# sulaimanvesal/PointCloudUDA

Measured on AMD Instinct MI355X. Metric: adversarial train-step images/sec (seg+3 discr) at 256x256, higher is better.
Workload: dtype bf16x3 MFMA (split-bf16, fp32 accumulate; fp32 storage); 1 GPU; MS-CMRSeg full UDA: UNet(PointNet head) + d1 + d2 + d4, 256x256x1, 4 classes; per_gpu_batch=32, global_batch=32, precision=bf16x3, parallelism=dp1, ranks_in_group=1, collective=none, streams=discriminators concurrent, d_target_forward=replayed from the adversarial pass of the same step, launch=eager (256 host cores for this rank)

## Files before the change

### pointcloududa_amd/csrc/conv_host.h

```cpp
#pragma once
#include <stdlib.h>
#include <string.h>
#include "conv_igemm.h"

static const int LDS_HARD = 160 * 1024;

static inline bool geom_ok(const pcuda_conv_geom* g) {
  if (!g || g->n <= 0 || g->cin <= 0 || g->cout <= 0 || g->k <= 0 || g->stride <= 0 || g->dil <= 0 || g->pad < 0)
    return false;
  if (g->k * g->k > IG_MAX_TAPS) return false;
  const int oh = (g->in_h + 2 * g->pad - g->dil * (g->k - 1) - 1) / g->stride + 1;
  const int ow = (g->in_w + 2 * g->pad - g->dil * (g->k - 1) - 1) / g->stride + 1;
  if (oh != g->out_h || ow != g->out_w || oh <= 0 || ow <= 0) return false;
  if (g->in_up && ((g->in_h & 1) || (g->in_w & 1))) return false;
  return true;
}

static inline bool src_ok(const pcuda_src* s, int c) {
  if (!s || !s->p1 || s->c1 <= 0 || s->c1 > c) return false;
  if (s->c1 < c && !s->p2) return false;
  return true;
}
static inline bool dst_ok(const pcuda_dst* d, int c) {
  if (!d || !d->p1 || d->c1 <= 0 || d->c1 > c) return false;
// ... 75 lines not shown

static inline int tile_width_candidates(int lw, int tile_px, int* out) {
  int n = 0;
  for (int t = 8; t <= 256 && t <= tile_px; t <<= 1) out[n++] = t;
  for (int parts = 1; parts <= 4; ++parts) {
    const int t = (lw + parts - 1) / parts;
    if (t >= 4 && t <= 256 && t <= tile_px) {
      bool dup = false;
      for (int i = 0; i < n; ++i) dup |= out[i] == t;
      if (!dup) out[n++] = t;
    }
  }
  return n;
}


static inline bool fast_src_ok(const pcuda_src* x, int cin) {
  const long long lim = 1ll << 30;
  const int c1 = x->c1 < cin ? x->c1 : cin;
  if (c1 < cin && (c1 & 31)) return false;
  if ((long long)(c1 + 32) * x->sc1 * 4 >= lim) return false;
  if (c1 < cin && (long long)(cin - c1 + 32) * x->sc2 * 4 >= lim) return false;
  return true;
}

static inline bool fast_dst_ok(const pcuda_dst* y, int cout) {
  const long long lim = 1ll << 30;
  const int c1 = y->c1 < cout ? y->c1 : cout;
  if (c1 < cout && (c1 & 7)) return false;
  if ((long long)(c1 + 64) * y->sc1 * 4 >= lim) return false;
  if (c1 < cout && (long long)(cout - c1 + 64) * y->sc2 * 4 >= lim) return false;
  return true;
}

struct IgemmPlan {
  int npb, tw, th, tiles_x, tiles_y, ih_t, iw_t, clamp, x_cap, tg;
  size_t lds;
  int fat;
  int w8;
  int te;
};

static inline bool te_dst_ok(const pcuda_dst* y, int cout, int out_w, int lw, int tw, int ox_mul, int ox_off) {
  if (ox_mul != 1 || ox_off != 0 || (tw & 3) || (out_w & 3) || (lw & 3)) return false;
  if (((uintptr_t)y->p1 & 15) || (y->sc1 & 3) || (y->sn1 & 3)) return false;
  if (y->c1 < cout && (((uintptr_t)y->p2 & 15) || (y->sc2 & 3) || (y->sn2 & 3))) return false;
  return true;
}


struct IgemmParams;
struct PackParams;
bool ap_layer_ok(const pcuda_conv_geom* g, int rows, int red, int prec);
size_t ap_layer_packed_bytes(int rows, int red);
bool ap_fill_pack(PackParams& p, const float* w, unsigned char* out, int rows, int red, long long s_row, long long s_red,
                  const TapSet& taps);
int ap_launch_pack(const float* w, unsigned char* out, int rows, int red, long long s_row, long long s_red, const TapSet& taps,
                   hipStream_t s);
bool ap_map_ok(int n, int h, int w, int rows);
int ap_tiles(int n, int h, int w);
int ap_try_launch(const IgemmParams& p, const TapSet& taps, const unsigned char* image, hipStream_t s, int* rc);

bool rs_layer_ok(const pcuda_conv_geom* g, int rows, int red, int prec);
bool rs_map_ok(int n, int h, int w);
int rs_tiles(int n, int h, int w);
int rs_try_launch(const IgemmParams& p, int prec, const TapSet& taps, hipStream_t s, int* rc);

int direct_fwd_tiles(const pcuda_conv_geom* g);
int direct_forward(const pcuda_conv_geom* g, int prec, const pcuda_src* x, const void* packed_w, long long w_lo_off,
                   const float* bias, float slope, const pcuda_dst* y, float* bn_partials, hipStream_t s, int* rc);
int direct_dgrad_tiles(const pcuda_conv_geom* g);
int direct_dgrad(const pcuda_conv_geom* g, int prec, const pcuda_src* dy, const void* packed_w_dgrad, const pcuda_dst* dx,
                 int accumulate, hipStream_t s, int* rc, const float* red_a = nullptr, long long red_sn = 0,
                 long long red_sc = 0, const float* red_mean = nullptr, const float* red_invstd = nullptr,
                 float* red = nullptr);
size_t direct_wgrad_workspace(const pcuda_conv_geom* g);
int direct_wgrad(const pcuda_conv_geom* g, const pcuda_src* x, const float* dz, long long dz_sn, long long dz_sc, float* dw,
                 float* db, int accumulate, void* workspace, hipStream_t s, int* rc);
int direct_d1_dgrad(const pcuda_conv_geom* g, int prec, const pcuda_src* dy, const void* packed_w_dgrad, const pcuda_dst* dx,
                    int accumulate, size_t cls_elems, hipStream_t s, int* rc);
size_t direct_d1_wgrad_workspace(const pcuda_conv_geom* g);
int direct_d1_wgrad(const pcuda_conv_geom* g, const pcuda_src* x, const float* dz, long long dz_sn, long long dz_sc, float* dw,
                    float* db, int accumulate, void* workspace, hipStream_t s, int* rc);
int launch_wgrad_reduce_taps(const float* partial, long long numel, int ksplit, float* dw, int accumulate, int ntaps,
                             const float* db_partial, long long nb, float* db, hipStream_t s);
size_t wgrad3r_workspace(const pcuda_conv_geom* g);
int wgrad3r_try(const pcuda_conv_geom* g, int prec, const pcuda_src* x, const float* dy, long long dy_sn, long long dy_sc,
                float* dw, float* db, int accumulate, void* workspace, hipStream_t s, pcuda_reduce_job* defer, int* rc);
size_t wgrad1_workspace(const pcuda_conv_geom* g);
int wgrad1_try(const pcuda_conv_geom* g, int prec, const pcuda_src* x, const float* dy, long long dy_sn, long long dy_sc,
               float* dw, float* db, int accumulate, void* workspace, hipStream_t s, pcuda_reduce_job* defer, int* rc);
size_t wgrad3_workspace(const pcuda_conv_geom* g);
int wgrad3_try(const pcuda_conv_geom* g, int prec, const pcuda_src* x, const float* dy, long long dy_sn, long long dy_sc,
               float* dw, float* db, int accumulate, void* workspace, hipStream_t s, pcuda_reduce_job* defer, int* rc);
int launch_wgrad_reduce(const float* partial, long long numel, int ksplit, float* dw, int accumulate, const float* db_partial,
                        long long nb, float* db, hipStream_t s);
int direct_d1_forward(const pcuda_conv_geom* g, int prec, const pcuda_src* x, const void* packed_w, const float* bias,
                      float slope, const pcuda_dst* y, float* bn_partials, hipStream_t s, int* rc);
int direct_d5_forward(const pcuda_conv_geom* g, int prec, const pcuda_src* x, const void* packed_w, const float* bias,
                      float slope, const pcuda_dst* y, float* bn_partials, hipStream_t s, int* rc);
```

### pointcloududa_amd/csrc/conv_wgrad.hip

```cpp
#include "conv_igemm.h"
#include "conv_host.h"

__global__ __launch_bounds__(1024) void wgrad_reduce_kernel(const float* __restrict__ partial, long long numel,
                                                           int ksplit, float* __restrict__ dw, int accumulate,
                                                           int ntaps, const float* __restrict__ db_partial,
                                                           long long nb, float* __restrict__ db) {
  __shared__ float sh[16][64];
  const int lane = threadIdx.x & 63, kg = threadIdx.x >> 6, nkg = blockDim.x >> 6;
  const long long nblk_w = (numel + 63) / 64;
  long long blk = blockIdx.x;
  if (blk >= nblk_w) {
    blk -= nblk_w; partial = db_partial; numel = nb; dw = db; ntaps = 1;
  }
  const long long i = blk * 64 + lane;
  float s = 0.f;
  if (i < numel) {
    int k = kg;
    for (; k + 7 * nkg < ksplit; k += 8 * nkg) {
      float v[8];
#pragma unroll
      for (int u = 0; u < 8; ++u) v[u] = partial[(long long)(k + u * nkg) * numel + i];
#pragma unroll
      for (int u = 0; u < 8; ++u) s += v[u];
    }
    for (; k < ksplit; k += nkg) s += partial[(long long)k * numel + i];
  }
  sh[kg][lane] = s;
  __syncthreads();
  if (kg == 0 && i < numel) {
    float t = 0.f;
    for (int q = 0; q < nkg; ++q) t += sh[q][lane];
    long long o = i;
    if (ntaps > 1) {
      const long long cc = numel / ntaps;
      const long long tt = i / cc, r = i - tt * cc;
      o = r * ntaps + tt;
    }
    dw[o] = accumulate ? dw[o] + t : t;
  }
}

int launch_wgrad_reduce_taps(const float* partial, long long numel, int ksplit, float* dw, int accumulate, int ntaps,
                             const float* db_partial, long long nb, float* db, hipStream_t s) {
  int nkg = 1;
  while (nkg < 16 && nkg * 2 <= ksplit) nkg <<= 1;
  const unsigned nblk = (unsigned)cdiv(numel, 64) + (db ? (unsigned)cdiv(nb, 64) : 0u);
  hipLaunchKernelGGL(wgrad_reduce_kernel, dim3(nblk), dim3(64 * nkg), 0, s, partial, numel, ksplit, dw, accumulate, ntaps,
                     db_partial, db ? nb : 0, db);
  PCUDA_CHECK_LAUNCH("wgrad_reduce_kernel");
  return PCUDA_OK;
}
int launch_wgrad_reduce(const float* partial, long long numel, int ksplit, float* dw, int accumulate, const float* db_partial,
                        long long nb, float* db, hipStream_t s) {
  return launch_wgrad_reduce_taps(partial, numel, ksplit, dw, accumulate, 1, db_partial, nb, db, s);
}

struct ReduceJobs {
  int n;
  int first_block[PCUDA_REDUCE_MAX_JOBS + 1];
  pcuda_reduce_job j[PCUDA_REDUCE_MAX_JOBS];
};

__global__ __launch_bounds__(1024) void wgrad_reduce_batch_kernel(const ReduceJobs jobs) {
  __shared__ float sh[16][64];
  int lo = 0, hi = jobs.n - 1;
  while (lo < hi) {
    const int mid = (lo + hi + 1) >> 1;
    if (jobs.first_block[mid] <= (int)blockIdx.x) lo = mid; else hi = mid - 1;
  }
  const pcuda_reduce_job& jb = jobs.j[lo];
  const float* partial = jb.partial;
  long long numel = jb.numel;
  float* dw = jb.dw;
  int ntaps = jb.ntaps;
  const int ksplit = jb.ksplit, nkg = jb.nkg;
  const int lane = threadIdx.x & 63, kg = threadIdx.x >> 6;
  const long long nblk_w = (numel + 63) / 64;
  long long blk = (int)blockIdx.x - jobs.first_block[lo];
  if (blk >= nblk_w) { blk -= nblk_w; partial = jb.db_partial; numel = jb.nb; dw = jb.db; ntaps = 1; }
  const long long i = blk * 64 + lane;
  float s = 0.f;
  if (i < numel && kg < nkg) {
    int k = kg;
    for (; k + 7 * nkg < ksplit; k += 8 * nkg) {
      float v[8];
#pragma unroll
      for (int u = 0; u < 8; ++u) v[u] = partial[(long long)(k + u * nkg) * numel + i];
#pragma unroll
      for (int u = 0; u < 8; ++u) s += v[u];
    }
    for (; k < ksplit; k += nkg) s += partial[(long long)k * numel + i];
  }
  sh[kg][lane] = s;
  __syncthreads();
  if (kg == 0 && i < numel) {
    float t = 0.f;
    for (int q = 0; q < nkg; ++q) t += sh[q][lane];
    long long o = i;
    if (ntaps > 1) {
      const long long cc = numel / ntaps;
      const long long tt = i / cc, r = i - tt * cc;
      o = r * ntaps + tt;
    }
    dw[o] = jb.accumulate ? dw[o] + t : t;
  }
}

extern "C" int pcuda_wgrad_reduce_batch(const pcuda_reduce_job* host_jobs, int njobs, pcuda_stream_t s) {
  if (!host_jobs || njobs < 0) PCUDA_FAIL(PCUDA_E_BADARG, "wgrad_reduce_batch: bad arguments");
  int done = 0;
  while (done < njobs) {
    ReduceJobs jobs;
    jobs.n = 0;
    int blocks = 0;
    for (; done < njobs && jobs.n < PCUDA_REDUCE_MAX_JOBS; ++done) {
      const pcuda_reduce_job& jb = host_jobs[done];
      if (jb.ksplit <= 0) continue;
      if (!jb.partial || !jb.dw || jb.numel <= 0 || jb.nkg < 1 || jb.nkg > 16 || (jb.db && !jb.db_partial))
        PCUDA_FAIL(PCUDA_E_BADARG, "wgrad_reduce_batch: bad job %d", done);
      jobs.first_block[jobs.n] = blocks;
      jobs.j[jobs.n++] = jb;
      blocks += (int)cdiv(jb.numel, 64) + (jb.db ? (int)cdiv(jb.nb, 64) : 0);
    }
    if (jobs.n == 0) break;
    jobs.first_block[jobs.n] = blocks;
    ProfScope prof(PCUDA_FAM_POINTWISE, 0.0, (hipStream_t)s, "wgrad reduce batch");
    hipLaunchKernelGGL(wgrad_reduce_batch_kernel, dim3(blocks), dim3(1024), 0, (hipStream_t)s, jobs);
    PCUDA_CHECK_LAUNCH("wgrad_reduce_batch_kernel");
  }
  return PCUDA_OK;
}

namespace {

struct WgradPlan {
  int co_blks, co_tile, n_co_tiles, n_chunks, tap_groups, taps_per_group, tw, th, tiles_x, tiles_y, ksplit;
  int ih_t, iw_t;
};

WgradPlan plan_wgrad(const pcuda_conv_geom* g) {
  WgradPlan w;
  w.co_blks = ig_co_blks(g->cout);
  w.co_tile = 32 * w.co_blks;
  w.n_co_tiles = cdiv(g->cout, w.co_tile);
  w.n_chunks = cdiv(g->cin, 32);
  const int ntaps = g->k * g->k;
  w.tap_groups = ntaps <= 16 ? 1 : cdiv(ntaps, 9);
  w.taps_per_group = cdiv(ntaps, w.tap_groups);
  {
    int cand[16];
    const int nc = tile_width_candidates(g->out_w, 128, cand);
    long long best_key = -1;
    w.tw = 32; w.th = 4;
    for (int ci = 0; ci < nc; ++ci) {
      const int tw = cand[ci], th = 128 / tw;
      if (th < 1) continue;
      const int span = (g->k - 1) * g->dil;
      const long long halo = (long long)((th - 1) * g->stride + span + 1) * ((tw - 1) * g->stride + span + 1);
      {
        const long long ih = (th - 1) * g->stride + span + 1, iw = (tw - 1) * g->stride + span + 1;
        const long long clipped = (ih < g->in_h ? ih : g->in_h) * (iw < g->in_w ? iw : g->in_w) + 1;
        const long long cap = halo < clipped ? halo : clipped;
        if (cap * IG_REC_BYTES * 2 + (long long)w.co_tile * WG_ZROW * 2 > (long long)LDS_HARD) continue;
      }
      const long long ih2 = (th - 1) * g->stride + span + 1, iw2 = (tw - 1) * g->stride + span + 1;
      const long long clipped2 = (ih2 < g->in_h ? ih2 : g->in_h) * (iw2 < g->in_w ? iw2 : g->in_w) + 1;
      const long long staged = (clipped2 * 2 <= halo) ? clipped2 : halo;
      const long long key = ((long long)cdiv(g->out_w, tw) * cdiv(g->out_h, th) << 24) + (staged > 768 ? (1ll << 22) : 0) +
                            ((tw & 31) ? (1ll << 20) : 0) + halo;
      if (best_key < 0 || key < best_key) { best_key = key; w.tw = tw; w.th = th; }
    }
  }
  const int TW = w.tw, TH = w.th;
  w.tiles_x = cdiv(g->out_w, TW);
  w.tiles_y = cdiv(g->out_h, TH);
  const int span = (g->k - 1) * g->dil;
  w.ih_t = (TH - 1) * g->stride + span + 1;
  w.iw_t = (TW - 1) * g->stride + span + 1;
  const long long ntiles = (long long)g->n * w.tiles_x * w.tiles_y;
  const int base = w.n_co_tiles * w.n_chunks * w.tap_groups;
  static int tgt32 = -1;
  if (tgt32 < 0) { const char* e = getenv("PCUDA_WG_BLOCKS32"); tgt32 = e ? atoi(e) : 768; }
  static int tgt64 = -1;
  if (tgt64 < 0) { const char* e = getenv("PCUDA_WG_BLOCKS64"); tgt64 = e ? atoi(e) : 1024; }
  static int tgt1 = -1;
  if (tgt1 < 0) { const char* e = getenv("PCUDA_WG_BLOCKS1"); tgt1 = e ? atoi(e) : 256; }
  bool one_per_cu = false;
  {
    const long long full = (long long)w.ih_t * w.iw_t;
    const long long clipped = (long long)(w.ih_t < g->in_h ? w.ih_t : g->in_h) * (w.iw_t < g->in_w ? w.iw_t : g->in_w) + 1;
    const size_t zb = (size_t)w.co_tile * WG_ZROW * 2;
    bool clamp = clipped * 2 <= full;
    if (!clamp && (size_t)full * IG_REC_BYTES * 2 + zb > (size_t)LDS_HARD) clamp = true;
    one_per_cu = (size_t)(clamp ? clipped : full) * IG_REC_BYTES * 2 + zb > (size_t)LDS_HARD / 2;
  }
  long long ks = (one_per_cu ? tgt1 : (w.co_blks == 1 ? tgt32 : tgt64)) / base;
  if (ks < 1) ks = 1;
  if (ks > ntiles) ks = ntiles;
  const long long welems = (long long)g->cout * g->cin * ntaps;
  while (ks > 1 && ks * welems * 4 > (64ll << 20)) ks >>= 1;
  if (ks >= 8) ks &= ~7ll;
  w.ksplit = (int)ks;
  return w;
}

}

extern "C" size_t pcuda_conv2d_wgrad_workspace_size(const pcuda_conv_geom* g) {
  if (!geom_ok(g)) return 0;
  WgradPlan w = plan_wgrad(g);
// ... 45 lines not shown
               pcuda_conv2d_wgrad_workspace_size(g));
  {
    int rc;
    if (direct_wgrad(g, x, dy, dy_sn, dy_sc, dw, db, accumulate, workspace, s, &rc)) return rc;
    if (direct_d1_wgrad(g, x, dy, dy_sn, dy_sc, dw, db, accumulate, workspace, s, &rc)) return rc;
    if (wgrad3r_try(g, prec, x, dy, dy_sn, dy_sc, dw, db, accumulate, workspace, s, defer, &rc)) return rc;
    if (wgrad3_try(g, prec, x, dy, dy_sn, dy_sc, dw, db, accumulate, workspace, s, defer, &rc)) return rc;
    if (wgrad1_try(g, prec, x, dy, dy_sn, dy_sc, dw, db, accumulate, workspace, s, defer, &rc)) return rc;
  }
  const bool x3 = prec == PCUDA_PREC_BF16X3;
  WgradPlan w = plan_wgrad(g);
  TapSet t = fwd_taps(g);
  WgradParams p;
  memset(&p, 0, sizeof(p));
  p.x = *x; p.cin = g->cin;
  p.in_h = g->in_h; p.in_w = g->in_w; p.in_shift = g->in_up ? 1 : 0; p.in_row = g->in_w >> p.in_shift;
  p.dz = dy; p.dz_sn = dy_sn; p.dz_sc = dy_sc;
  p.cout = g->cout; p.out_h = g->out_h; p.out_w = g->out_w;
  p.stride = g->stride;
  p.ntaps = w.taps_per_group; p.ntaps_total = t.n; p.tap_groups = w.tap_groups;
  memcpy(p.dy, t.dy, sizeof(p.dy));
  memcpy(p.dx, t.dx, sizeof(p.dx));
  p.dy_min = t.dy_min; p.dx_min = t.dx_min;
  p.ih_t = w.ih_t; p.iw_t = w.iw_t;
  p.tw = w.tw; p.th = w.th; p.tmagic = 65536 / w.tw + 1; p.tiles_x = w.tiles_x; p.tiles_y = w.tiles_y; p.n = g->n;
  p.ksplit = w.ksplit; p.n_co_tiles = w.n_co_tiles; p.n_chunks = w.n_chunks;
  p.partial = (float*)workspace;
  {
    static int dbg = -1;
    if (dbg < 0) { const char* e = getenv("PCUDA_DBG"); dbg = e ? atoi(e) : 0; }
    p.dbg = dbg;
  }
  p.tw16 = ((w.tw & 15) == 0 && w.tw * w.th == 128) ? 1 : 0;
  p.aligned4 = ((g->out_w & 7) == 0 && (w.tw & 7) == 0 && (dy_sn & 3) == 0 && (dy_sc & 3) == 0 && (((uintptr_t)dy) & 15) == 0 &&
                ((long long)g->cout * dy_sc + (long long)g->out_h * g->out_w) * 4 < (1ll << 30)) ? 1 : 0;
  const long long welems = (long long)g->cout * g->cin * t.n;
  float* dbp = db ? (float*)workspace + (size_t)w.ksplit * welems : nullptr;

  const int full = w.ih_t * w.iw_t;
  const int clipped = (w.ih_t < g->in_h ? w.ih_t : g->in_h) * (w.iw_t < g->in_w ? w.iw_t : g->in_w) + 1;
  const size_t mul = x3 ? 2 : 1;
  const size_t zb = (size_t)w.co_tile * WG_ZROW * mul;
  bool clamp = clipped * 2 <= full;
  if (!clamp && (size_t)full * IG_REC_BYTES * mul + zb > (size_t)LDS_HARD) clamp = true;
  const int x_cap = clamp ? clipped : full;
  const size_t lds = (size_t)x_cap * IG_REC_BYTES * mul + zb;
  if (lds > (size_t)LDS_HARD) PCUDA_FAIL(PCUDA_E_UNSUPPORTED, "conv2d_wgrad: tile %dx%d does not fit LDS", w.ih_t, w.iw_t);
  const dim3 grid(w.n_co_tiles * w.n_chunks * w.tap_groups, w.ksplit);
  {
    static int noxcd = -1;
    if (noxcd < 0) { const char* e = getenv("PCUDA_WG_NOXCD"); noxcd = (e && atoi(e)) ? 1 : 0; }
    const long long nblk = (long long)grid.x * grid.y;
    p.xcd_items = (!noxcd && nblk >= 16 && (nblk & 7) == 0) ? (int)(nblk / 8) : 0;
    static int nointer = -1;
    if (nointer < 0) { const char* e = getenv("PCUDA_WG_NOINTER"); nointer = (e && atoi(e)) ? 1 : 0; }
    p.xcd_slices = (p.xcd_items && !nointer && (w.ksplit & 7) == 0) ? w.ksplit / 8 : 0;
  }
  {
    const double flops = 2.0 * g->n * (double)g->out_h * g->out_w * g->cout * (double)g->cin * t.n;
    char tag[160];
    static int nopipe = -1;
    if (nopipe < 0) { const char* e = getenv("PCUDA_NOPIPE"); nopipe = (e && atoi(e)) ? 1 : 0; }
    int pf = (nopipe || !fast_src_ok(x, g->cin)) ? 0 : (x_cap <= 256 ? 1 : (x_cap <= 768 ? 3 : 0));
    static int now8 = -1;
    if (now8 < 0) { const char* e = getenv("PCUDA_WG_NO8"); now8 = (e && atoi(e)) ? 1 : 0; }
    if (!now8 && pf > 0 && w.taps_per_group > 9 && x_cap <= 1024) pf = 100 + (x_cap <= 512 ? 1 : 2);
    {
      static int noxq = -1;
      if (noxq < 0) { const char* e = getenv("PCUDA_NOXQ"); noxq = e ? atoi(e) : 0; }
      const int slots = pf >= 100 ? pf - 100 : pf, per = pf >= 100 ? 128 : 64;
      const int ih = clamp ? (w.ih_t < g->in_h ? w.ih_t : g->in_h) : w.ih_t;
      const int in_w_phys = g->in_up ? g->in_w / 2 : g->in_w;
      p.xq = (!noxq && slots > 0 && !g->in_up && (in_w_phys & 3) == 0 && (ih * ((w.iw_t + 6) / 4) + per - 1) / per <= slots) ? 1 : 0;
    }
    snprintf(tag, sizeof(tag), "wgrad n%d cin%d cout%d %dx%d k%d s%d d%d ksplit%d clamp%d pf%d lds%zu", g->n, g->cin,
             g->cout, g->out_h, g->out_w, g->k, g->stride, g->dil, w.ksplit, clamp ? 1 : 0, pf, lds);
    ProfScope prof(PCUDA_FAM_CONV_WGRAD, flops, s, tag);
    int rc;
    const int taps_max = w.taps_per_group <= 1 ? 1 : w.taps_per_group <= 9 ? 9 : 16;
    rc = x3 ? wgrad_dispatch_x3(p, w.co_blks, clamp, taps_max, pf, x_cap, lds, dbp, grid, s)
            : wgrad_dispatch_bf16(p, w.co_blks, clamp, taps_max, pf, x_cap, lds, dbp, grid, s);
    if (rc) return rc;
  }
  {
    int nkg = 1;
    while (nkg < 16 && nkg * 2 <= w.ksplit) nkg <<= 1;
    if (defer) {
      defer->partial = (const float*)workspace; defer->numel = welems; defer->ksplit = w.ksplit; defer->nkg = nkg;
      defer->dw = dw; defer->accumulate = accumulate; defer->ntaps = t.n;
      defer->db_partial = (const float*)dbp; defer->nb = db ? g->cout : 0; defer->db = db;
      return PCUDA_OK;
    }
    const unsigned nblk = (unsigned)cdiv(welems, 64) + (db ? (unsigned)cdiv(g->cout, 64) : 0u);
    hipLaunchKernelGGL(wgrad_reduce_kernel, dim3(nblk), dim3(64 * nkg), 0, s, (const float*)workspace, welems, w.ksplit,
                       dw, accumulate, t.n, (const float*)dbp, (long long)(db ? g->cout : 0), db);
    PCUDA_CHECK_LAUNCH("wgrad_reduce_kernel");
  }
  return PCUDA_OK;
}
```

### pointcloududa_amd/csrc/conv_wgrad1.hip

```cpp
#include "conv_device.h"
#include "conv_host.h"

namespace {

struct W1Params {
  pcuda_src x;
  int cin, cout, n;
  int hw;
  const float* dz; long long dz_sn, dz_sc;
  float* partial;
  float* db_partial;
  int steps_per_wg;
  int wgs_per_image;
  int n_ci_tiles, tiles;
  int xcd;
};

template <int NB>
struct W1Raw {
  f32x4 v[NB][2];
};

template <bool X3, int CO_B, int CI_B>
__global__ __launch_bounds__(256, 2) void wgrad1_kernel(const W1Params p) {
// ... 168 lines not shown
  static int off = -1;
  if (off < 0) { const char* e = getenv("PCUDA_NO_WGRAD1"); off = (e && atoi(e)) ? 1 : 0; }
  if (off) return false;
  const long long hw = (long long)g->in_h * g->in_w;
  return g->k == 1 && g->stride == 1 && g->pad == 0 && !g->in_up && (hw & 15) == 0 && hw < (1ll << 28) && g->cin >= 16;
}

W1Plan w1_plan(const pcuda_conv_geom* g) {
  W1Plan w;
  w.co_b = g->cout > 32 ? 2 : 1;
  w.ci_b = g->cin > 64 ? 3 : (g->cin > 32 ? 2 : 1);
  w.n_co_tiles = cdiv(g->cout, 32 * w.co_b);
  w.n_ci_tiles = cdiv(g->cin, 32 * w.ci_b);
  const int tiles = w.n_co_tiles * w.n_ci_tiles;
  const long long spi = (long long)g->in_h * g->in_w / 16, total = spi * g->n;
  static int tgt = -1;
  if (tgt < 0) { const char* e = getenv("PCUDA_WG1_BLOCKS"); tgt = e ? atoi(e) : 768; }
  long long want = tgt / tiles;
  const long long welems = (long long)g->cout * g->cin;
  const long long in_bytes = total * 16 * (g->cin + g->cout) * 4;
  long long cap = in_bytes / 8;
  if (cap < (8ll << 20)) cap = 8ll << 20;
  if (want * welems * 4 > cap) want = cap / (welems * 4);
  if (want > total / 8) want = total / 8;
  if (want < 1) want = 1;
  long long d = cdiv(total, want);
  if (d > spi) d = spi;
  while (spi % d) ++d;
  w.steps_per_wg = (int)d;
  w.wgs_per_image = (int)(spi / d);
  w.slices = w.wgs_per_image * g->n;
  return w;
}

}

size_t wgrad1_workspace(const pcuda_conv_geom* g) {
  if (!w1_geom(g)) return 0;
  const W1Plan w = w1_plan(g);
  return ((size_t)w.slices * g->cout * g->cin + (size_t)w.slices * g->cout) * sizeof(float) + 256;
}

int wgrad1_try(const pcuda_conv_geom* g, int prec, const pcuda_src* x, const float* dy, long long dy_sn, long long dy_sc,
               float* dw, float* db, int accumulate, void* workspace, hipStream_t s, pcuda_reduce_job* defer, int* rc) {
  if (!w1_geom(g)) return 0;
  auto al = [](const void* q, long long sn, long long sc) { return q == nullptr || ((((uintptr_t)q) & 15) == 0 && (sn & 3) == 0 && (sc & 3) == 0); };
  const int c1 = x->c1 < g->cin ? x->c1 : g->cin;
  if (!al(x->p1, x->sn1, x->sc1) || (c1 < g->cin && !al(x->p2, x->sn2, x->sc2)) || !al(dy, dy_sn, dy_sc)) return 0;
  const bool x3 = prec == PCUDA_PREC_BF16X3;
  const W1Plan w = w1_plan(g);
  W1Params p;
  memset(&p, 0, sizeof(p));
  p.x = *x; p.x.c1 = c1;
  p.cin = g->cin; p.cout = g->cout; p.n = g->n; p.hw = g->in_h * g->in_w;
  p.dz = dy; p.dz_sn = dy_sn; p.dz_sc = dy_sc;
  const long long welems = (long long)g->cout * g->cin;
  p.partial = (float*)workspace;
  p.db_partial = db ? (float*)workspace + (size_t)w.slices * welems : nullptr;
  p.steps_per_wg = w.steps_per_wg; p.wgs_per_image = w.wgs_per_image;
  p.n_ci_tiles = w.n_ci_tiles; p.tiles = w.n_co_tiles * w.n_ci_tiles;
  const long long nwg = (long long)p.tiles * w.slices;
  if (nwg >= (1ll << 31)) return 0;
  p.xcd = (nwg >= 16 && (nwg & 7) == 0) ? 1 : 0;
  {
    char tag[160];
    snprintf(tag, sizeof(tag), "wgrad1 n%d cin%d cout%d %dx%d k1 slices%d steps%d tile%dx%d", g->n, g->cin, g->cout, g->in_h,
             g->in_w, w.slices, w.steps_per_wg, 32 * w.co_b, 32 * w.ci_b);
    ProfScope prof(PCUDA_FAM_CONV_WGRAD, 2.0 * g->n * (double)p.hw * g->cout * (double)g->cin, s, tag);
    const dim3 grid((unsigned)nwg);
#define W1_LAUNCH(X3_, CO_, CI_) hipLaunchKernelGGL((wgrad1_kernel<X3_, CO_, CI_>), grid, dim3(256), 0, s, p)
#define W1_CI(X3_, CO_)                                                \
  do {                                                                 \
    if (w.ci_b == 3) W1_LAUNCH(X3_, CO_, 3);                           \
    else if (w.ci_b == 2) W1_LAUNCH(X3_, CO_, 2);                      \
    else W1_LAUNCH(X3_, CO_, 1);                                       \
  } while (0)
    if (x3) { if (w.co_b == 2) W1_CI(true, 2); else W1_CI(true, 1); }
    else { if (w.co_b == 2) W1_CI(false, 2); else W1_CI(false, 1); }
#undef W1_CI
#undef W1_LAUNCH
    hipError_t e = hipGetLastError();
    if (e != hipSuccess) { pcuda_set_error("wgrad1_kernel: %s", hipGetErrorString(e)); *rc = PCUDA_E_LAUNCH; return 1; }
  }
  int nkg = 1;
  while (nkg < 16 && nkg * 2 <= w.slices) nkg <<= 1;
  if (defer) {
    defer->partial = (const float*)workspace; defer->numel = welems; defer->ksplit = w.slices; defer->nkg = nkg;
    defer->dw = dw; defer->accumulate = accumulate; defer->ntaps = 1;
    defer->db_partial = (const float*)p.db_partial; defer->nb = db ? g->cout : 0; defer->db = db;
    *rc = PCUDA_OK;
    return 1;
  }
  *rc = launch_wgrad_reduce_taps((const float*)workspace, welems, w.slices, dw, accumulate, 1, (const float*)p.db_partial,
                                 db ? g->cout : 0, db, s);
  return 1;
}
```

### pointcloududa_amd/csrc/conv_wgrad3.hip

```cpp
#include "conv_device.h"
#include "conv_host.h"

namespace {

constexpr int W3_TW = 32, W3_TH = 4;
constexpr int W3_XW = 40;
constexpr int W3_XROWS = W3_TH + 2;
constexpr int W3_XREC = W3_XW * W3_XROWS;
constexpr int W3_XPLANE = W3_XREC * IG_REC_BYTES;
constexpr int W3_ITEMS = W3_XROWS * (W3_XW / 4);

struct W3Params {
  pcuda_src x;
  int cin, H, W;
  const float* dz; long long dz_sn, dz_sc;
  int cout;
  int tiles_x, tiles_y, n;
  int ksplit, n_chunks;
  float* partial;
  float* db_partial;
  int base, xcd;
  int dbg;
};

// ... 293 lines not shown
  return true;
}

W3Plan w3_plan(const pcuda_conv_geom* g) {
  W3Plan w;
  w.rb = 2;
  w.kh = 1;
  w.n_co_tiles = g->cout / (32 * w.rb);
  w.n_chunks = g->cin / 32;
  w.tiles_x = g->out_w / W3_TW;
  w.tiles_y = g->out_h / W3_TH;
  const long long ntiles = (long long)g->n * w.tiles_x * w.tiles_y;
  const int base = w.n_co_tiles * w.n_chunks;
  static int tgt = -1;
  if (tgt < 0) { const char* e = getenv("PCUDA_WG3_BLOCKS"); tgt = e ? atoi(e) : 1024; }
  long long ks = tgt / base;
  if (ks < 1) ks = 1;
  if (ks > ntiles) ks = ntiles;
  const long long welems = (long long)g->cout * g->cin * 9;
  while (ks > 1 && ks * w.kh * welems * 4 > (64ll << 20)) ks >>= 1;
  if (ks >= 8) ks &= ~7ll;
  w.ksplit = (int)ks;
  return w;
}

}

size_t wgrad3_workspace(const pcuda_conv_geom* g) {
  if (g->k != 3 || g->stride != 1 || g->dil != 1 || g->pad != 1 || g->in_up || (g->out_w % W3_TW) || (g->out_h % W3_TH) ||
      (g->cout & 63) || (g->cin & 31))
    return 0;
  const W3Plan w = w3_plan(g);
  return ((size_t)w.ksplit * w.kh * g->cout * g->cin * 9 + (size_t)w.ksplit * w.kh * g->cout) * sizeof(float) + 256;
}

int wgrad3_try(const pcuda_conv_geom* g, int prec, const pcuda_src* x, const float* dy, long long dy_sn, long long dy_sc,
               float* dw, float* db, int accumulate, void* workspace, hipStream_t s, pcuda_reduce_job* defer, int* rc) {
  if (!w3_eligible(g, x, dy, dy_sn, dy_sc)) return 0;
  const bool x3 = prec == PCUDA_PREC_BF16X3;
  const W3Plan w = w3_plan(g);
  W3Params p;
  memset(&p, 0, sizeof(p));
  p.x = *x; p.cin = g->cin; p.H = g->in_h; p.W = g->in_w;
  p.dz = dy; p.dz_sn = dy_sn; p.dz_sc = dy_sc; p.cout = g->cout;
  p.tiles_x = w.tiles_x; p.tiles_y = w.tiles_y; p.n = g->n;
  p.ksplit = w.ksplit; p.n_chunks = w.n_chunks;
  {
    static int dbg = -1;
    if (dbg < 0) { const char* e = getenv("PCUDA_W3DBG"); dbg = e ? atoi(e) : 0; }
    p.dbg = dbg;
  }
  const int slices = w.ksplit * w.kh;
  const long long welems = (long long)g->cout * g->cin * 9;
  p.partial = (float*)workspace;
  p.db_partial = db ? (float*)workspace + (size_t)slices * welems : nullptr;
  const size_t lds = (size_t)(x3 ? 2 : 1) * (W3_XPLANE + 32 * w.rb * WG_ZROW);
  p.base = w.n_co_tiles * w.n_chunks;
  {
    static int noxcd = -1;
    if (noxcd < 0) { const char* e = getenv("PCUDA_W3_NOXCD"); noxcd = (e && atoi(e)) ? 1 : 0; }
    p.xcd = (!noxcd && (w.ksplit % 8) == 0) ? 1 : 0;
  }
  const dim3 grid(p.base * w.ksplit);
  {
    char tag[160];
    snprintf(tag, sizeof(tag), "wgrad3 n%d cin%d cout%d %dx%d k3 s1 d1 ksplit%d rb%d lds%zu", g->n, g->cin, g->cout, g->out_h,
             g->out_w, w.ksplit, w.rb, lds);
    ProfScope prof(PCUDA_FAM_CONV_WGRAD, 2.0 * g->n * (double)g->out_h * g->out_w * g->cout * (double)g->cin * 9, s, tag);
#define W3_LAUNCH(X3_, RB_, KH_)                                                                                       \
  do {                                                                                                                  \
    auto kern = wgrad3_kernel<X3_, RB_, KH_>;                                                                          \
    if (lds > 48 * 1024) {                  \
      hipError_t e = hipFuncSetAttribute((const void*)kern, hipFuncAttributeMaxDynamicSharedMemorySize, (int)LDS_HARD); \
      if (e != hipSuccess) { pcuda_set_error("wgrad3: cannot raise dynamic LDS: %s", hipGetErrorString(e)); *rc = PCUDA_E_LAUNCH; return 1; } \
    }                                                                                                                   \
    hipLaunchKernelGGL(kern, grid, dim3(64 * RB_ * 2 * KH_), lds, s, p);                                                \
  } while (0)
    if (x3) W3_LAUNCH(true, 2, 1);
    else W3_LAUNCH(false, 2, 1);
#undef W3_LAUNCH
    hipError_t e = hipGetLastError();
    if (e != hipSuccess) { pcuda_set_error("wgrad3_kernel: %s", hipGetErrorString(e)); *rc = PCUDA_E_LAUNCH; return 1; }
  }
  int nkg = 1;
  while (nkg < 16 && nkg * 2 <= slices) nkg <<= 1;
  if (defer) {
    defer->partial = (const float*)workspace; defer->numel = welems; defer->ksplit = slices; defer->nkg = nkg;
    defer->dw = dw; defer->accumulate = accumulate; defer->ntaps = 9;
    defer->db_partial = (const float*)p.db_partial; defer->nb = db ? g->cout : 0; defer->db = db;
    *rc = PCUDA_OK;
    return 1;
  }
  *rc = launch_wgrad_reduce_taps((const float*)workspace, welems, slices, dw, accumulate, 9, (const float*)p.db_partial,
                                 db ? g->cout : 0, db, s);
  return 1;
}
```

### pointcloududa_amd/csrc/conv_wgrad3r.hip

```cpp
#include <type_traits>

#include "conv_device.h"
#include "conv_host.h"

namespace {

struct W3RParams {
  pcuda_src x;
  int cin, cout, n, H, W;
  const float* dz; long long dz_sn, dz_sc;
  float* partial;
  float* db_partial;
  int n_ci_tiles, tiles;
  int strips;
  int rsplit;
  int npairs;
  int pairs_per_slice;
  int xcd;
  int dbg;
};

struct RowF {
  uint4 f[3][2];
};
// ... 267 lines not shown
  if (maxc < 0) { const char* e = getenv("PCUDA_W3R_MAXC"); maxc = e ? atoi(e) : 128; }
  static int upmaxc = -1;
  if (upmaxc < 0) { const char* e = getenv("PCUDA_W3R_UPMAXC"); upmaxc = e ? atoi(e) : 512; }
  const int mc = (g->in_up && upmaxc > maxc) ? upmaxc : maxc;
  const bool shape = g->k == 3 && g->stride == 1 && g->pad == 1 && g->dil == 1 && (g->in_w & 31) == 0 && g->in_h >= 4 &&
                     (!g->in_up || (g->in_h & 1) == 0) &&
                     g->cin >= 16 && g->cin <= mc && g->cout <= mc && (long long)g->in_h * g->in_w < (1ll << 28);
  if (!shape || mode >= 2) return shape;
  if (g->in_up) return g->cin <= upmaxc && g->cout <= upmaxc;
  if (g->in_h >= 128 && g->in_w >= 128) return true;
  return g->cin != g->cout && g->cin <= 64 && g->cout <= 64 && g->in_h >= 64;
}

W3RPlan w3r_plan(const pcuda_conv_geom* g) {
  W3RPlan w;
  w.n_co_tiles = cdiv(g->cout, 32);
  w.n_ci_tiles = cdiv(g->cin, 32);
  const int tiles = w.n_co_tiles * w.n_ci_tiles;
  w.strips = g->in_w / 32;
  w.rsplit = 1;
  while ((long long)g->n * w.strips * w.rsplit * tiles < 256 && g->in_h / (w.rsplit * 2) >= 32) w.rsplit *= 2;
  w.npairs = g->n * w.strips * w.rsplit;
  static int tgt = -1;
  if (tgt < 0) { const char* e = getenv("PCUDA_W3R_BLOCKS"); tgt = e ? atoi(e) : 512; }
  long long want = tgt / tiles;
  const long long welems = (long long)g->cout * g->cin * 9;
  if (want * welems * 4 > (32ll << 20)) want = (32ll << 20) / (welems * 4);
  if (want < 1) want = 1;
  if (want > w.npairs) want = w.npairs;
  w.pairs_per_slice = cdiv(w.npairs, (int)want);
  w.slices = cdiv(w.npairs, w.pairs_per_slice);
  return w;
}

}

size_t wgrad3r_workspace(const pcuda_conv_geom* g) {
  if (!w3r_geom(g)) return 0;
  const W3RPlan w = w3r_plan(g);
  return ((size_t)w.slices * g->cout * g->cin * 9 + (size_t)w.slices * g->cout) * sizeof(float) + 256;
}

int wgrad3r_try(const pcuda_conv_geom* g, int prec, const pcuda_src* x, const float* dy, long long dy_sn, long long dy_sc,
                float* dw, float* db, int accumulate, void* workspace, hipStream_t s, pcuda_reduce_job* defer, int* rc) {
  if (!w3r_geom(g)) return 0;
  auto al = [](const void* q, long long sn, long long sc) { return q == nullptr || ((((uintptr_t)q) & 15) == 0 && (sn & 3) == 0 && (sc & 3) == 0); };
  const int c1 = x->c1 < g->cin ? x->c1 : g->cin;
  if (!al(x->p1, x->sn1, x->sc1) || (c1 < g->cin && !al(x->p2, x->sn2, x->sc2)) || !al(dy, dy_sn, dy_sc)) return 0;
  const bool x3 = prec == PCUDA_PREC_BF16X3;
  const W3RPlan w = w3r_plan(g);
  W3RParams p;
  memset(&p, 0, sizeof(p));
  p.x = *x; p.x.c1 = c1;
  p.cin = g->cin; p.cout = g->cout; p.n = g->n; p.H = g->in_h; p.W = g->in_w;
  p.dz = dy; p.dz_sn = dy_sn; p.dz_sc = dy_sc;
  const long long welems = (long long)g->cout * g->cin * 9;
  p.partial = (float*)workspace;
  p.db_partial = db ? (float*)workspace + (size_t)w.slices * welems : nullptr;
  p.n_ci_tiles = w.n_ci_tiles; p.tiles = w.n_co_tiles * w.n_ci_tiles;
  p.strips = w.strips; p.rsplit = w.rsplit; p.npairs = w.npairs; p.pairs_per_slice = w.pairs_per_slice;
  const long long nwg = (long long)p.tiles * w.slices;
  p.xcd = (nwg >= 16 && (nwg & 7) == 0) ? 1 : 0;
  {
    static int dbg = -1;
    if (dbg < 0) { const char* e = getenv("PCUDA_W3RDBG"); dbg = e ? atoi(e) : 0; }
    p.dbg = dbg;
  }
  {
    char tag[160];
    snprintf(tag, sizeof(tag), "wgrad3r n%d cin%d cout%d %dx%d k3 s1 d1 up%d slices%d pairs%d", g->n, g->cin, g->cout, g->in_h, g->in_w,
             g->in_up ? 1 : 0, w.slices, w.pairs_per_slice);
    ProfScope prof(PCUDA_FAM_CONV_WGRAD, 2.0 * g->n * (double)g->in_h * g->in_w * g->cout * (double)g->cin * 9, s, tag);
    const dim3 grid((unsigned)nwg);
    if (g->in_up) {
      if (x3) hipLaunchKernelGGL((wgrad3r_kernel<true, true>), grid, dim3(256), 0, s, p);
      else hipLaunchKernelGGL((wgrad3r_kernel<false, true>), grid, dim3(256), 0, s, p);
    } else {
      if (x3) hipLaunchKernelGGL(wgrad3r_kernel<true>, grid, dim3(256), 0, s, p);
      else hipLaunchKernelGGL(wgrad3r_kernel<false>, grid, dim3(256), 0, s, p);
    }
    hipError_t e = hipGetLastError();
    if (e != hipSuccess) { pcuda_set_error("wgrad3r_kernel: %s", hipGetErrorString(e)); *rc = PCUDA_E_LAUNCH; return 1; }
  }
  int nkg = 1;
  while (nkg < 16 && nkg * 2 <= w.slices) nkg <<= 1;
  if (defer) {
    defer->partial = (const float*)workspace; defer->numel = welems; defer->ksplit = w.slices; defer->nkg = nkg;
    defer->dw = dw; defer->accumulate = accumulate; defer->ntaps = 9;
    defer->db_partial = (const float*)p.db_partial; defer->nb = db ? g->cout : 0; defer->db = db;
    *rc = PCUDA_OK;
    return 1;
  }
  *rc = launch_wgrad_reduce_taps((const float*)workspace, welems, w.slices, dw, accumulate, 9, (const float*)p.db_partial,
                                 db ? g->cout : 0, db, s);
  return 1;
}
```

Measured before the change: 755.7 img/s.

## Rewrite wgrad split-K reduction with tiled LDS transpose and vectorized loads

```diff
diff --git a/pointcloududa_amd/csrc/conv_host.h b/pointcloududa_amd/csrc/conv_host.h
--- a/pointcloududa_amd/csrc/conv_host.h
+++ b/pointcloududa_amd/csrc/conv_host.h
@@ -181,6 +181,11 @@
 size_t direct_d1_wgrad_workspace(const pcuda_conv_geom* g);
 int direct_d1_wgrad(const pcuda_conv_geom* g, const pcuda_src* x, const float* dz, long long dz_sn, long long dz_sc, float* dw,
                     float* db, int accumulate, void* workspace, hipStream_t s, int* rc);
+static inline int wgrad_reduce_nkg(int ksplit) {
+  int nkg = 1;
+  while (nkg < 16 && nkg * 2 <= ksplit) nkg <<= 1;
+  return nkg;
+}
 int launch_wgrad_reduce_taps(const float* partial, long long numel, int ksplit, float* dw, int accumulate, int ntaps,
                              const float* db_partial, long long nb, float* db, hipStream_t s);
 size_t wgrad3r_workspace(const pcuda_conv_geom* g);
diff --git a/pointcloududa_amd/csrc/conv_wgrad.hip b/pointcloududa_amd/csrc/conv_wgrad.hip
--- a/pointcloududa_amd/csrc/conv_wgrad.hip
+++ b/pointcloududa_amd/csrc/conv_wgrad.hip
@@ -1,52 +1,152 @@
 #include "conv_igemm.h"
 #include "conv_host.h"
 
-__global__ __launch_bounds__(1024) void wgrad_reduce_kernel(const float* __restrict__ partial, long long numel,
-                                                           int ksplit, float* __restrict__ dw, int accumulate,
-                                                           int ntaps, const float* __restrict__ db_partial,
-                                                           long long nb, float* __restrict__ db) {
-  __shared__ float sh[16][64];
-  const int lane = threadIdx.x & 63, kg = threadIdx.x >> 6, nkg = blockDim.x >> 6;
-  const long long nblk_w = (numel + 63) / 64;
-  long long blk = blockIdx.x;
-  if (blk >= nblk_w) {
-    blk -= nblk_w; partial = db_partial; numel = nb; dw = db; ntaps = 1;
-  }
-  const long long i = blk * 64 + lane;
-  float s = 0.f;
-  if (i < numel) {
-    int k = kg;
-    for (; k + 7 * nkg < ksplit; k += 8 * nkg) {
-      float v[8];
-#pragma unroll
-      for (int u = 0; u < 8; ++u) v[u] = partial[(long long)(k + u * nkg) * numel + i];
-#pragma unroll
-      for (int u = 0; u < 8; ++u) s += v[u];
+#define RED_THREADS 256
+#define RED_LDS_FLOATS 10240
+#define RED_PAD 4
+
+struct RedShape { int R, TT; };
+
+__host__ __device__ static inline long long red_shape_tiles(long long cc, int ntaps, RedShape t) {
+  return ((cc + t.R - 1) / t.R) * (ntaps / t.TT);
+}
+__host__ __device__ static inline bool red_whole_taps_bad(long long cc, int ntaps, int nkg, int R) {
+  return (long long)nkg * ntaps * (R + RED_PAD) > RED_LDS_FLOATS || (cc + R - 1) / R < 256;
+}
+__host__ __device__ static inline RedShape red_shape(long long cc, int ntaps, int nkg, int ksplit) {
+  RedShape t;
+  t.R = 256; t.TT = ntaps;
+  if (ntaps > 1) {
+    while (t.R > 32 && red_whole_taps_bad(cc, ntaps, nkg, t.R)) t.R >>= 1;
+    if (red_whole_taps_bad(cc, ntaps, nkg, t.R)) t.TT = 1;
+  }
+  if (t.TT == 1) {
+    t.R = 256;
+    while (t.R > 64 && ((cc + t.R - 1) / t.R) * ntaps < 512) t.R >>= 1;
+  }
+  return t;
+}
+__host__ __device__ static inline long long red_blocks(long long numel, int ntaps, int nkg, int ksplit) {
+  const long long cc = numel / ntaps;
+  return red_shape_tiles(cc, ntaps, red_shape(cc, ntaps, nkg, ksplit));
+}
+static inline size_t red_lds_bytes(long long numel, int ntaps, int nkg, int ksplit) {
+  const RedShape t = red_shape(numel / ntaps, ntaps, nkg, ksplit);
+  return (size_t)nkg * t.TT * (t.R + RED_PAD) * sizeof(float);
+}
+
+template <int VEC, int U, int S>
+__device__ __forceinline__ void red_group_sums(const float* __restrict__ partial, long long numel, long long cc, int ksplit,
+                                               int nkg, int nsteps, long long r0, int t0, int R, int TT, float* sh) {
+  const int RP = R + RED_PAD, rvn = R / VEC, rshift = __builtin_ctz(rvn), V = TT * rvn, P = nkg * V;
+  const long long sstride = (long long)nkg * numel;
+  for (int w0 = threadIdx.x; w0 < P; w0 += RED_THREADS * U) {
+    const float* p[U];
+    int q[U], lds[U];
+    bool ok[U];
+    float acc[U][VEC];
+#pragma unroll
+    for (int u = 0; u < U; ++u) {
+      const int w = w0 + u * RED_THREADS;
+      const int qq = w / V, item = w - qq * V, tt = item >> rshift, rv = item - (tt << rshift);
+      const long long pos = r0 + (long long)rv * VEC;
+      ok[u] = w < P && pos < cc;
+      q[u] = qq;
+      lds[u] = (qq * TT + tt) * RP + rv * VEC;
+      p[u] = partial + (long long)qq * numel + (long long)(t0 + tt) * cc + pos;
+#pragma unroll
+      for (int e = 0; e < VEC; ++e) acc[u][e] = 0.f;
     }
-    for (; k < ksplit; k += nkg) s += partial[(long long)k * numel + i];
-  }
-  sh[kg][lane] = s;
+    for (int s0 = 0; s0 < nsteps; s0 += S) {
+      float v[U][S][VEC];
+#pragma unroll
+      for (int u = 0; u < U; ++u)
+#pragma unroll
+        for (int ss = 0; ss < S; ++ss) {
+          const bool in = ok[u] && q[u] + (s0 + ss) * nkg < ksplit;
+          const float* a = in ? p[u] + (long long)(s0 + ss) * sstride : partial;
+          if constexpr (VEC == 4) {
+            const float4 t = *reinterpret_cast<const float4*>(a);
+            v[u][ss][0] = t.x; v[u][ss][1] = t.y; v[u][ss][2] = t.z; v[u][ss][3] = t.w;
+          } else {
+            v[u][ss][0] = *a;
+          }
+        }
+#pragma unroll
+      for (int u = 0; u < U; ++u)
+#pragma unroll
+        for (int ss = 0; ss < S; ++ss) {
+          const bool in = ok[u] && q[u] + (s0 + ss) * nkg < ksplit;
+#pragma unroll
+          for (int e = 0; e < VEC; ++e) acc[u][e] = in ? acc[u][e] + v[u][ss][e] : acc[u][e];
+        }
+    }
+#pragma unroll
+    for (int u = 0; u < U; ++u)
+      if (ok[u]) {
+        if constexpr (VEC == 4) *reinterpret_cast<float4*>(sh + lds[u]) = make_float4(acc[u][0], acc[u][1], acc[u][2], acc[u][3]);
+        else sh[lds[u]] = acc[u][0];
+      }
+  }
+}
+
+template <int VEC>
+__device__ __forceinline__ void red_group_sums_by_steps(const float* __restrict__ partial, long long numel, long long cc,
+                                                        int ksplit, int nkg, long long r0, int t0, int R, int TT, float* sh) {
+  const int nsteps = (ksplit + nkg - 1) / nkg;
+  if (nsteps <= 1) red_group_sums<VEC, 8, 1>(partial, numel, cc, ksplit, nkg, nsteps, r0, t0, R, TT, sh);
+  else if (nsteps == 2) red_group_sums<VEC, 4, 2>(partial, numel, cc, ksplit, nkg, nsteps, r0, t0, R, TT, sh);
+  else if (nsteps <= 4) red_group_sums<VEC, 2, 4>(partial, numel, cc, ksplit, nkg, nsteps, r0, t0, R, TT, sh);
+  else if (nsteps <= 8) red_group_sums<VEC, 1, 8>(partial, numel, cc, ksplit, nkg, nsteps, r0, t0, R, TT, sh);
+  else red_group_sums<VEC, 1, 16>(partial, numel, cc, ksplit, nkg, nsteps, r0, t0, R, TT, sh);
+}
+
+__device__ __forceinline__ void red_tile(const float* __restrict__ partial, long long numel, int ksplit, int nkg,
+                                         float* __restrict__ dw, int accumulate, int ntaps, long long blk, float* sh) {
+  const long long cc = numel / ntaps;
+  const RedShape ts = red_shape(cc, ntaps, nkg, ksplit);
+  const int R = ts.R, TT = ts.TT;
+  const long long rblks = (cc + R - 1) / R;
+  const long long tb = blk / rblks, rb = blk - tb * rblks;
+  const long long r0 = rb * R;
+  const int t0 = (int)tb * TT;
+  if ((((uintptr_t)partial) & 15) == 0 && (cc & 3) == 0) red_group_sums_by_steps<4>(partial, numel, cc, ksplit, nkg, r0, t0, R, TT, sh);
+  else red_group_sums_by_steps<1>(partial, numel, cc, ksplit, nkg, r0, t0, R, TT, sh);
   __syncthreads();
-  if (kg == 0 && i < numel) {
+  const int RP = R + RED_PAD;
+  const long long left = cc - r0;
+  const int nout = (int)(left < R ? left : R) * TT;
+  for (int o = threadIdx.x; o < nout; o += RED_THREADS) {
+    const int r = o / TT, tt = o - r * TT;
+    const long long gi = (r0 + r) * ntaps + t0 + tt;
+    const float old = accumulate ? dw[gi] : 0.f;
     float t = 0.f;
-    for (int q = 0; q < nkg; ++q) t += sh[q][lane];
-    long long o = i;
-    if (ntaps > 1) {
-      const long long cc = numel / ntaps;
-      const long long tt = i / cc, r = i - tt * cc;
-      o = r * ntaps + tt;
-    }
-    dw[o] = accumulate ? dw[o] + t : t;
-  }
+    for (int q = 0; q < nkg; ++q) t += sh[(q * TT + tt) * RP + r];
+    dw[gi] = accumulate ? old + t : t;
+  }
+}
+
+extern __shared__ __align__(16) float red_sh[];
+
+__global__ __launch_bounds__(RED_THREADS) void wgrad_reduce_kernel(const float* __restrict__ partial, long long numel,
+                                                                   int ksplit, int nkg, float* __restrict__ dw, int accumulate,
+                                                                   int ntaps, const float* __restrict__ db_partial,
+                                                                   long long nb, float* __restrict__ db) {
+  const long long nblk_w = red_blocks(numel, ntaps, nkg, ksplit);
+  const long long blk = blockIdx.x;
+  if (blk < nblk_w) red_tile(partial, numel, ksplit, nkg, dw, accumulate, ntaps, blk, red_sh);
+  else red_tile(db_partial, nb, ksplit, nkg, db, accumulate, 1, blk - nblk_w, red_sh);
 }
 
 int launch_wgrad_reduce_taps(const float* partial, long long numel, int ksplit, float* dw, int accumulate, int ntaps,
                              const float* db_partial, long long nb, float* db, hipStream_t s) {
-  int nkg = 1;
-  while (nkg < 16 && nkg * 2 <= ksplit) nkg <<= 1;
-  const unsigned nblk = (unsigned)cdiv(numel, 64) + (db ? (unsigned)cdiv(nb, 64) : 0u);
-  hipLaunchKernelGGL(wgrad_reduce_kernel, dim3(nblk), dim3(64 * nkg), 0, s, partial, numel, ksplit, dw, accumulate, ntaps,
-                     db_partial, db ? nb : 0, db);
+  if (ntaps < 1) ntaps = 1;
+  const int nkg = wgrad_reduce_nkg(ksplit);
+  const long long nblk = red_blocks(numel, ntaps, nkg, ksplit) + (db ? red_blocks(nb, 1, nkg, ksplit) : 0);
+  size_t lds = red_lds_bytes(numel, ntaps, nkg, ksplit);
+  if (db && red_lds_bytes(nb, 1, nkg, ksplit) > lds) lds = red_lds_bytes(nb, 1, nkg, ksplit);
+  hipLaunchKernelGGL(wgrad_reduce_kernel, dim3((unsigned)nblk), dim3(RED_THREADS), lds, s, partial, numel, ksplit, nkg, dw,
+                     accumulate, ntaps, db_partial, db ? nb : 0, db);
   PCUDA_CHECK_LAUNCH("wgrad_reduce_kernel");
   return PCUDA_OK;
 }
@@ -61,49 +161,18 @@
   pcuda_reduce_job j[PCUDA_REDUCE_MAX_JOBS];
 };
 
-__global__ __launch_bounds__(1024) void wgrad_reduce_batch_kernel(const ReduceJobs jobs) {
-  __shared__ float sh[16][64];
+__global__ __launch_bounds__(RED_THREADS) void wgrad_reduce_batch_kernel(const ReduceJobs jobs) {
   int lo = 0, hi = jobs.n - 1;
   while (lo < hi) {
     const int mid = (lo + hi + 1) >> 1;
     if (jobs.first_block[mid] <= (int)blockIdx.x) lo = mid; else hi = mid - 1;
   }
   const pcuda_reduce_job& jb = jobs.j[lo];
-  const float* partial = jb.partial;
-  long long numel = jb.numel;
-  float* dw = jb.dw;
-  int ntaps = jb.ntaps;
-  const int ksplit = jb.ksplit, nkg = jb.nkg;
-  const int lane = threadIdx.x & 63, kg = threadIdx.x >> 6;
-  const long long nblk_w = (numel + 63) / 64;
-  long long blk = (int)blockIdx.x - jobs.first_block[lo];
-  if (blk >= nblk_w) { blk -= nblk_w; partial = jb.db_partial; numel = jb.nb; dw = jb.db; ntaps = 1; }
-  const long long i = blk * 64 + lane;
-  float s = 0.f;
-  if (i < numel && kg < nkg) {
-    int k = kg;
-    for (; k + 7 * nkg < ksplit; k += 8 * nkg) {
-      float v[8];
-#pragma unroll
-      for (int u = 0; u < 8; ++u) v[u] = partial[(long long)(k + u * nkg) * numel + i];
-#pragma unroll
-      for (int u = 0; u < 8; ++u) s += v[u];
-    }
-    for (; k < ksplit; k += nkg) s += partial[(long long)k * numel + i];
-  }
-  sh[kg][lane] = s;
-  __syncthreads();
-  if (kg == 0 && i < numel) {
-    float t = 0.f;
-    for (int q = 0; q < nkg; ++q) t += sh[q][lane];
-    long long o = i;
-    if (ntaps > 1) {
-      const long long cc = numel / ntaps;
-      const long long tt = i / cc, r = i - tt * cc;
-      o = r * ntaps + tt;
-    }
-    dw[o] = jb.accumulate ? dw[o] + t : t;
-  }
+  const int ntaps = jb.ntaps < 1 ? 1 : jb.ntaps;
+  const long long nblk_w = red_blocks(jb.numel, ntaps, jb.nkg, jb.ksplit);
+  const long long blk = (int)blockIdx.x - jobs.first_block[lo];
+  if (blk < nblk_w) red_tile(jb.partial, jb.numel, jb.ksplit, jb.nkg, jb.dw, jb.accumulate, ntaps, blk, red_sh);
+  else red_tile(jb.db_partial, jb.nb, jb.ksplit, jb.nkg, jb.db, jb.accumulate, 1, blk - nblk_w, red_sh);
 }
 
 extern "C" int pcuda_wgrad_reduce_batch(const pcuda_reduce_job* host_jobs, int njobs, pcuda_stream_t s) {
@@ -112,20 +181,28 @@
   while (done < njobs) {
     ReduceJobs jobs;
     jobs.n = 0;
-    int blocks = 0;
+    long long blocks = 0;
+    size_t lds = 0;
     for (; done < njobs && jobs.n < PCUDA_REDUCE_MAX_JOBS; ++done) {
       const pcuda_reduce_job& jb = host_jobs[done];
       if (jb.ksplit <= 0) continue;
-      if (!jb.partial || !jb.dw || jb.numel <= 0 || jb.nkg < 1 || jb.nkg > 16 || (jb.db && !jb.db_partial))
+      const int ntaps = jb.ntaps < 1 ? 1 : jb.ntaps;
+      if (!jb.partial || !jb.dw || jb.numel <= 0 || jb.numel % ntaps != 0 || jb.nkg < 1 || jb.nkg > 16 ||
+          (jb.db && (!jb.db_partial || jb.nb <= 0)))
         PCUDA_FAIL(PCUDA_E_BADARG, "wgrad_reduce_batch: bad job %d", done);
-      jobs.first_block[jobs.n] = blocks;
+      const long long nblk = red_blocks(jb.numel, ntaps, jb.nkg, jb.ksplit) + (jb.db ? red_blocks(jb.nb, 1, jb.nkg, jb.ksplit) : 0);
+      if (blocks + nblk > 0x7fffffffll) PCUDA_FAIL(PCUDA_E_BADARG, "wgrad_reduce_batch: job %d is too large", done);
+      jobs.first_block[jobs.n] = (int)blocks;
       jobs.j[jobs.n++] = jb;
-      blocks += (int)cdiv(jb.numel, 64) + (jb.db ? (int)cdiv(jb.nb, 64) : 0);
+      blocks += nblk;
+      size_t l = red_lds_bytes(jb.numel, ntaps, jb.nkg, jb.ksplit);
+      if (l > lds) lds = l;
+      if (jb.db && (l = red_lds_bytes(jb.nb, 1, jb.nkg, jb.ksplit)) > lds) lds = l;
     }
     if (jobs.n == 0) break;
-    jobs.first_block[jobs.n] = blocks;
+    jobs.first_block[jobs.n] = (int)blocks;
     ProfScope prof(PCUDA_FAM_POINTWISE, 0.0, (hipStream_t)s, "wgrad reduce batch");
-    hipLaunchKernelGGL(wgrad_reduce_batch_kernel, dim3(blocks), dim3(1024), 0, (hipStream_t)s, jobs);
+    hipLaunchKernelGGL(wgrad_reduce_batch_kernel, dim3((unsigned)blocks), dim3(RED_THREADS), lds, (hipStream_t)s, jobs);
     PCUDA_CHECK_LAUNCH("wgrad_reduce_batch_kernel");
   }
   return PCUDA_OK;
@@ -337,19 +414,12 @@
             : wgrad_dispatch_bf16(p, w.co_blks, clamp, taps_max, pf, x_cap, lds, dbp, grid, s);
     if (rc) return rc;
   }
-  {
-    int nkg = 1;
-    while (nkg < 16 && nkg * 2 <= w.ksplit) nkg <<= 1;
-    if (defer) {
-      defer->partial = (const float*)workspace; defer->numel = welems; defer->ksplit = w.ksplit; defer->nkg = nkg;
-      defer->dw = dw; defer->accumulate = accumulate; defer->ntaps = t.n;
-      defer->db_partial = (const float*)dbp; defer->nb = db ? g->cout : 0; defer->db = db;
-      return PCUDA_OK;
-    }
-    const unsigned nblk = (unsigned)cdiv(welems, 64) + (db ? (unsigned)cdiv(g->cout, 64) : 0u);
-    hipLaunchKernelGGL(wgrad_reduce_kernel, dim3(nblk), dim3(64 * nkg), 0, s, (const float*)workspace, welems, w.ksplit,
-                       dw, accumulate, t.n, (const float*)dbp, (long long)(db ? g->cout : 0), db);
-    PCUDA_CHECK_LAUNCH("wgrad_reduce_kernel");
-  }
-  return PCUDA_OK;
-}
+  if (defer) {
+    defer->partial = (const float*)workspace; defer->numel = welems; defer->ksplit = w.ksplit; defer->nkg = wgrad_reduce_nkg(w.ksplit);
+    defer->dw = dw; defer->accumulate = accumulate; defer->ntaps = t.n;
+    defer->db_partial = (const float*)dbp; defer->nb = db ? g->cout : 0; defer->db = db;
+    return PCUDA_OK;
+  }
+  return launch_wgrad_reduce_taps((const float*)workspace, welems, w.ksplit, dw, accumulate, t.n, (const float*)dbp,
+                                  db ? g->cout : 0, db, s);
+}
diff --git a/pointcloududa_amd/csrc/conv_wgrad1.hip b/pointcloududa_amd/csrc/conv_wgrad1.hip
--- a/pointcloududa_amd/csrc/conv_wgrad1.hip
+++ b/pointcloududa_amd/csrc/conv_wgrad1.hip
@@ -274,10 +274,8 @@
     hipError_t e = hipGetLastError();
     if (e != hipSuccess) { pcuda_set_error("wgrad1_kernel: %s", hipGetErrorString(e)); *rc = PCUDA_E_LAUNCH; return 1; }
   }
-  int nkg = 1;
-  while (nkg < 16 && nkg * 2 <= w.slices) nkg <<= 1;
   if (defer) {
-    defer->partial = (const float*)workspace; defer->numel = welems; defer->ksplit = w.slices; defer->nkg = nkg;
+    defer->partial = (const float*)workspace; defer->numel = welems; defer->ksplit = w.slices; defer->nkg = wgrad_reduce_nkg(w.slices);
     defer->dw = dw; defer->accumulate = accumulate; defer->ntaps = 1;
     defer->db_partial = (const float*)p.db_partial; defer->nb = db ? g->cout : 0; defer->db = db;
     *rc = PCUDA_OK;
diff --git a/pointcloududa_amd/csrc/conv_wgrad3.hip b/pointcloududa_amd/csrc/conv_wgrad3.hip
--- a/pointcloududa_amd/csrc/conv_wgrad3.hip
+++ b/pointcloududa_amd/csrc/conv_wgrad3.hip
@@ -399,10 +399,8 @@
     hipError_t e = hipGetLastError();
     if (e != hipSuccess) { pcuda_set_error("wgrad3_kernel: %s", hipGetErrorString(e)); *rc = PCUDA_E_LAUNCH; return 1; }
   }
-  int nkg = 1;
-  while (nkg < 16 && nkg * 2 <= slices) nkg <<= 1;
   if (defer) {
-    defer->partial = (const float*)workspace; defer->numel = welems; defer->ksplit = slices; defer->nkg = nkg;
+    defer->partial = (const float*)workspace; defer->numel = welems; defer->ksplit = slices; defer->nkg = wgrad_reduce_nkg(slices);
     defer->dw = dw; defer->accumulate = accumulate; defer->ntaps = 9;
     defer->db_partial = (const float*)p.db_partial; defer->nb = db ? g->cout : 0; defer->db = db;
     *rc = PCUDA_OK;
diff --git a/pointcloududa_amd/csrc/conv_wgrad3r.hip b/pointcloududa_amd/csrc/conv_wgrad3r.hip
--- a/pointcloududa_amd/csrc/conv_wgrad3r.hip
+++ b/pointcloududa_amd/csrc/conv_wgrad3r.hip
@@ -373,10 +373,8 @@
     hipError_t e = hipGetLastError();
     if (e != hipSuccess) { pcuda_set_error("wgrad3r_kernel: %s", hipGetErrorString(e)); *rc = PCUDA_E_LAUNCH; return 1; }
   }
-  int nkg = 1;
-  while (nkg < 16 && nkg * 2 <= w.slices) nkg <<= 1;
   if (defer) {
-    defer->partial = (const float*)workspace; defer->numel = welems; defer->ksplit = w.slices; defer->nkg = nkg;
+    defer->partial = (const float*)workspace; defer->numel = welems; defer->ksplit = w.slices; defer->nkg = wgrad_reduce_nkg(w.slices);
     defer->dw = dw; defer->accumulate = accumulate; defer->ntaps = 9;
     defer->db_partial = (const float*)p.db_partial; defer->nb = db ? g->cout : 0; defer->db = db;
     *rc = PCUDA_OK;
```

After: 758.9 img/s, median of 6. About the same (+0.4%).
